# kav-institute/SemanticLiDARUnc

Measured on AMD Instinct MI355X. Metric: range-image scans/sec (64x2048, T=8 MC), higher is better.
Workload: dtype f16 (fp16 activations/weights, fp32 accumulate + epilogue, fp32 logits); 1 GPU; SalsaNext MC-dropout T=8 + entropy/MI map + IoU/ECE accumulation, 8 scans of 64x2048x5 per step per GPU (BASELINE configs[2] shape); T=8, parallelism=scan-sharded x1, mc_schedule=every pass fully recomputed

## Files before the change

semanticlidarunc_amd/csrc/conv2d_h8.hip:

```cpp
#include <stdio.h>
#include "h8_common.h"
#include <cstdlib>

#ifndef H8_M128_OPT_3X3
#define H8_M128_OPT_3X3 15
#endif
#ifndef H8_M128_OPT_2X2
#define H8_M128_OPT_2X2 15
#endif
#ifndef H8_M128_KPC2_DEFAULT
#define H8_M128_KPC2_DEFAULT 0
#endif

namespace {

struct H8Src {
  const uint4* ptr;
  const float* scale;
  int G;
  int gbeg;
  int nb;
  int shuf;
};

struct H8Args {
  H8Src src[SLU_MAX_SRC];
  int nsrc;
  int N, H, W, Gin, Cout, Gout, nmblk, nks;
  const uint4* wpack;
  const float *bias, *bn_a, *bn_b;
  int has_act;
  float slope;
  int out_f32;
  int tiles_x, tiles_y;
  int order;
#ifdef SLU_H8_AB
  int dbg;
#endif
};

struct SrcSel {
  const uint4* ptr;
  const float* scale;
  int G, gl, ns;
};

__device__ __forceinline__ SrcSel select_src(const H8Args& a, const int (&img)[SLU_MAX_SRC], int g) {
  SrcSel p{a.src[0].ptr, a.src[0].scale, a.src[0].G, g, img[0]};
#pragma unroll
  for (int s = 1; s < SLU_MAX_SRC; ++s)
    if (s < a.nsrc && g >= a.src[s].gbeg) p = SrcSel{a.src[s].ptr, a.src[s].scale, a.src[s].G, g - a.src[s].gbeg, img[s]};
  return p;
}

template <int STRIDE>
__device__ __forceinline__ void store_tile(const H8Args& a, const f32x16& acc, const float* se, int cl0, int co0, int hh, bool pix_ok,
                                           size_t n, size_t pix, size_t HW, const void* __restrict__ resid, void* __restrict__ out,
                                           float slope_pre) {
#pragma unroll
  for (int q = 0; q < 4; ++q) {
    float v[4];
#pragma unroll
    for (int k = 0; k < 4; ++k) {
      const int cl = cl0 + 8 * q + 4 * hh + k;
      float t = acc[4 * q + k] + se[cl];
      t = t > 0.0f ? t : t * slope_pre;
      v[k] = t * se[STRIDE + cl] + se[2 * STRIDE + cl];
    }
    const int co = co0 + 8 * q + 4 * hh;
    if (a.out_f32) {
      float* o = reinterpret_cast<float*>(out);
#pragma unroll
      for (int k = 0; k < 4; ++k)
        if (pix_ok && co + k < a.Cout) o[(n * a.Cout + co + k) * HW + pix] = v[k];
    } else {
      const int go = co >> 3;
      const bool ok = pix_ok && go < a.Gout;
      const size_t idx = ok ? ((n * a.Gout + go) * HW + pix) * 2 + hh : 0;
      if (resid) {
        const uint2 rv = reinterpret_cast<const uint2*>(resid)[idx];
        const half2v r0 = __builtin_bit_cast(half2v, rv.x), r1 = __builtin_bit_cast(half2v, rv.y);
        v[0] += (float)r0[0]; v[1] += (float)r0[1]; v[2] += (float)r1[0]; v[3] += (float)r1[1];
      }
      if (ok) reinterpret_cast<uint2*>(out)[idx] = make_uint2(pack2(v[0], v[1]), pack2(v[2], v[3]));
    }
  }
}

template <int STRIDE, bool PRE>
__device__ __forceinline__ void store_tile_full(const H8Args& a, const f32x16& acc, const float* se, int cl0, int go0, int hh, bool pix_ok, size_t n,
                                                size_t pix, size_t HW, const uint2* __restrict__ resid, const uint2 (&rv)[4],
                                                uint2* __restrict__ out, float slope_pre, uintptr_t zero_addr, uintptr_t trash_addr) {
  const float4* se4 = reinterpret_cast<const float4*>(se);
  const float2v sl = {slope_pre, slope_pre};
  const size_t plane2 = HW * 2;
  const size_t idx0 = ((n * a.Gout + go0) * HW + pix) * 2 + hh;
#pragma unroll
  for (int q = 0; q < 4; ++q) {
    const int c4 = (cl0 + 8 * q) / 4 + hh;
    H8Quad t = h8_epilogue(acc, q, se4[c4], se4[STRIDE / 4 + c4], se4[2 * STRIDE / 4 + c4], sl);
    const bool ok = pix_ok && go0 + q < a.Gout;
    const size_t idx = idx0 + q * plane2;
    if (resid) h8_add_resid(t, PRE ? rv[q] : *(ok ? resid + idx : reinterpret_cast<const uint2*>(zero_addr)));
    *(ok ? out + idx : reinterpret_cast<uint2*>(trash_addr)) = pack4(t);
  }
}

template <int STRIDE>
__device__ __forceinline__ void store_tile_swap16(const H8Args& a, const f32x16& acc, const float* se, int cl0, int go0, int hh, bool pix_ok, size_t n,
                                                  size_t pix, size_t HW, const uint2* __restrict__ resid, uint4* __restrict__ out, float slope_pre,
                                                  uintptr_t zero_addr, uintptr_t trash_addr) {
  const float4* se4 = reinterpret_cast<const float4*>(se);
  const float2v sl = {slope_pre, slope_pre};
#pragma unroll
  for (int pr = 0; pr < 2; ++pr) {
    unsigned hw[4];
#pragma unroll
    for (int q2 = 0; q2 < 2; ++q2) {
      const int q = 2 * pr + q2;
      const int c4 = (cl0 + 8 * q) / 4 + hh;
      H8Quad t = h8_epilogue(acc, q, se4[c4], se4[STRIDE / 4 + c4], se4[2 * STRIDE / 4 + c4], sl);
      if (resid) {
        const bool okq = pix_ok && go0 + q < a.Gout;
        h8_add_resid(t, *(okq ? resid + (((n * a.Gout + go0 + q) * HW + pix) * 2 + hh) : reinterpret_cast<const uint2*>(zero_addr)));
      }
      hw[2 * q2] = pack2(t.t0);
      hw[2 * q2 + 1] = pack2(t.t1);
    }
    const uint4 rec = h8_swap16(hw[0], hw[1], hw[2], hw[3]);
    const int go = go0 + 2 * pr + hh;
    *((pix_ok && go < a.Gout) ? out + ((n * a.Gout + go) * HW + pix) : reinterpret_cast<uint4*>(trash_addr)) = rec;
  }
}

#ifdef SLU_H8_PROF
__device__ unsigned long long g_h8_prof[8];
#define H8_PROF_MARK(i)                                         \
  {                                                             \
    const unsigned long long t_now = __builtin_amdgcn_s_memtime(); \
    asm volatile("" ::: "memory");                              \
    prof_acc[i] += t_now - prof_t;                              \
    prof_t = t_now;                                             \
  }
#else
#define H8_PROF_MARK(i)
#endif

constexpr int h8_waves_per_simd(int mb, int nwave, int rpw) { return (mb * rpw >= 8) ? 1 : ((nwave >= 8 || mb >= 2 || rpw >= 2) ? 2 : 3); }

template <int KS, int DIL, int PAD, int MB, int WM, int WN, int RPW, bool SCALED, bool WRES, bool F32OUT, int KPC = 1, int OPT = 0, bool ONE = false>
__global__ __launch_bounds__(64 * WM * WN, h8_waves_per_simd(MB, WM * WN, RPW)) void conv_h8_kernel(const H8Args a, const void* __restrict__ resid,
                                                                                                       void* __restrict__ out) {
  constexpr int NWAVE = WM * WN;
  constexpr int T = KS * KS, TS = KPC * T;
  constexpr int TW = 64, TH = WN * RPW, NB = 2 * RPW;
  constexpr int LW = TW + 2 * PAD, LH = TH + 2 * PAD;
  constexpr int REC = LH * LW;
  constexpr int MBLK = WM * MB;
  constexpr int NREC_B = KPC * 2 * REC, NBLK_B = (NREC_B + 63) / 64;
  constexpr int NB_ALLOC = NBLK_B * 64;
  constexpr int NREC_A = MBLK * TS * 64, NBLK_A = MBLK * TS;
  constexpr int NIB = (NBLK_B + NWAVE - 1) / NWAVE, NIA = (NBLK_A + NWAVE - 1) / NWAVE;
  static_assert(KPC == 1 || (!WRES && !SCALED && MB == 2 && WM == 2 && WN == 4), "multi-K-step chunks: the 8-wave 128-channel configuration only");
  static_assert(OPT == 0 || (MB == 2 && WM == 2 && WN == 4 && !F32OUT), "OPT: the 8-wave 128-channel configuration only");
  static_assert(KPC <= 2, "pc_rc carries 2 bits of channel block");
  static_assert(KPC == 1 || ONE, "multi-K-step chunks: single-source layers only");
  constexpr bool SHUF = SCALED && KS == 3 && DIL == 1 && PAD == 1 && !ONE && KPC == 1;
  static_assert(!SHUF || (WN * RPW) % 2 == 0, "tile rows start on even image rows");

  extern __shared__ __attribute__((aligned(16))) char smem[];
  float* s_epi = reinterpret_cast<float*>(smem);
  uint4* s_scale = reinterpret_cast<uint4*>(s_epi + 3 * MBLK * 32);
  uint4* s_b = s_scale + (SCALED ? 128 : 0);
  uint4* s_a = s_b + 2 * NB_ALLOC;

  const int tid = threadIdx.x, lane = tid & 63, wave = __builtin_amdgcn_readfirstlane(tid >> 6);
  const int wm = wave / WN, wn = wave % WN;
  const bool late_half = wave >= NWAVE / 2;
  const int mblk0 = blockIdx.y * MBLK;
  int t_beg, t_end, t_step = 1;
  {
    const int nwg = gridDim.x, b = blockIdx.x, xcd = b & 7, qq = nwg >> 3, rr = nwg & 7;
    const int w = (xcd < rr ? xcd * (qq + 1) : rr * (qq + 1) + (xcd - rr) * qq) + (b >> 3);
    const long long nt = (long long)a.tiles_x * a.tiles_y * a.N;
    if (a.order) {
      t_step = nwg;
      t_beg = w;
      t_end = w < nt ? w + (int)((nt - w + nwg - 1) / nwg) * nwg : w;
    } else {
      t_beg = (int)(nt * w / nwg);
      t_end = (int)(nt * (w + 1) / nwg);
    }
  }
  t_beg = __builtin_amdgcn_readfirstlane(t_beg);
  t_end = __builtin_amdgcn_readfirstlane(t_end);
  t_step = __builtin_amdgcn_readfirstlane(t_step);
  if (t_beg >= t_end) return;

  if (tid < MBLK * 32) {
    const int co = mblk0 * 32 + tid;
    const bool ok = co < a.Cout;
    H8_FILL_EPI(s_epi, 0, MBLK * 32, tid, ok, co, a.bias, a.bn_a, a.bn_b);
  }

  const int hh = lane >> 5, jj = lane & 31;
  const size_t HW = (size_t)a.H * a.W;
  const float slope_pre = (a.has_act & 3) == 1 ? a.slope : 1.0f;
  const int nks = a.nks;
  const int nchunk = (nks + KPC - 1) / KPC;
  const int a_stride = WRES ? nks * T * 64 : TS * 64;
  const int abase = (wm * MB) * a_stride + lane;
  const int bbase = hh * REC + (wn * RPW) * LW + jj;

  struct TilePos { int tx, ty, x0, y0, n, i0, i1, i2; };
  auto rfl = [](int v) __attribute__((always_inline)) { return __builtin_amdgcn_readfirstlane(v); };
  const int step_tx = rfl(t_step % a.tiles_x), step_ty = rfl((t_step / a.tiles_x) % a.tiles_y), step_n = rfl(t_step / (a.tiles_x * a.tiles_y));
  auto finish = [&](TilePos& p) __attribute__((always_inline)) {
    p.x0 = p.tx * TW;
    p.y0 = p.ty * TH;
    p.i0 = p.i1 = p.i2 = p.n;
    if constexpr (!ONE) {
      if (a.src[0].nb) p.i0 = rfl(p.n % a.src[0].nb);
      if (a.nsrc > 1 && a.src[1].nb) p.i1 = rfl(p.n % a.src[1].nb);
      if (a.nsrc > 2 && a.src[2].nb) p.i2 = rfl(p.n % a.src[2].nb);
    }
  };
  auto decode = [&](int t) __attribute__((always_inline)) {
    TilePos p;
    p.tx = rfl(t % a.tiles_x);
    t /= a.tiles_x;
    p.ty = rfl(t % a.tiles_y);
    p.n = rfl(t / a.tiles_y);
    finish(p);
    return p;
  };
  auto advance = [&](TilePos p) __attribute__((always_inline)) {
    p.tx += step_tx;
    if (p.tx >= a.tiles_x) p.tx -= a.tiles_x, p.ty += 1;
    p.ty += step_ty;
    if (p.ty >= a.tiles_y) p.ty -= a.tiles_y, p.n += 1;
    p.n += step_n;
    finish(p);
    return p;
  };
  static_assert(SLU_MAX_SRC == 3, "TilePos carries one image index per source");
  H8_OPAQUE_ADDR(zero_addr, h8_zero_rec);
  H8_OPAQUE_ADDR(trash_addr, h8_trash_rec);
  int pc_rc[NIB], pc_off[NIB];
#pragma unroll
  for (int i = 0; i < NIB; ++i) {
    const int e = (i * NWAVE + wave) * 64 + lane;
    const int g2 = e / REC;
    const int rem = e - g2 * REC;
    const int r = rem / LW;
    const int c = rem - r * LW;
    pc_rc[i] = r | (c << 8) | ((g2 & (2 * KPC - 1)) << 16) | ((e < NREC_B ? 1 : 0) << 20);
    pc_off[i] = r * a.W + c + (g2 & (2 * KPC - 1)) * (int)HW;
  }
  constexpr int NPIECE = NIB + (WRES ? 0 : NIA);
  constexpr int PPT = (NPIECE + TS - 1) / TS;
  uintptr_t st_b0 = 0, st_b1 = 0;
  bool st_sh = false;
  const int hw4 = (a.H >> 1) * (a.W >> 1), w2 = a.W >> 1;
  int st_g0 = 0;
  bool st_on = false;
  int st_x0 = 0, st_y0 = 0, st_q = 0, st_wave = wave;
  uint4 *st_db = s_b, *st_da = s_a;
  auto stage_begin = [&](const TilePos& tp, int q, int buf) __attribute__((always_inline)) {
    const int img[SLU_MAX_SRC] = {tp.i0, tp.i1, tp.i2};
    long long org = (long long)(tp.y0 - PAD) * a.W + (tp.x0 - PAD);
    st_g0 = 2 * KPC * q;
    if constexpr (SHUF) {
      st_sh = a.src[0].shuf && st_g0 < a.src[0].G;
      if (st_sh) org = 0;
    }
    if constexpr (ONE) {
      st_b0 = reinterpret_cast<uintptr_t>(a.src[0].ptr) + 16 * ((long long)(((size_t)tp.n * a.src[0].G + st_g0) * HW) + org);
      st_b1 = st_b0;
    } else {
      const SrcSel p0 = select_src(a, img, st_g0 < a.Gin ? st_g0 : 0), p1 = select_src(a, img, st_g0 + 1 < a.Gin ? st_g0 + 1 : 0);
      st_b0 = reinterpret_cast<uintptr_t>(p0.ptr) + 16 * ((long long)(((size_t)p0.ns * p0.G + p0.gl) * HW) + org);
      st_b1 = reinterpret_cast<uintptr_t>(p1.ptr) + 16 * ((long long)(((size_t)p1.ns * p1.G + p1.gl) * HW) + org - (long long)HW);
    }
    st_x0 = tp.x0 - PAD;
// ... 332 lines not shown
        x[ks][b] = ok ? v : make_uint4(0u, 0u, 0u, 0u);
      }
    }
    __syncthreads();
    H8_PROF_MARK(0)
    uint4 sw[NW];
#pragma unroll
    for (int i = 0; i < NW; ++i) {
      const int e = tid + i * 256;
      const int m = e / (KSPC * 64);
      const int r = e - m * (KSPC * 64);
      const int ks = r >> 6;
      const bool ok = (NWV % 256 == 0 || e < NWV) && m < a.nmblk && q * KSPC + ks < a.nks;
      const size_t off = ok ? ((size_t)m * a.nks + q * KSPC) * 64 + r : 0;
      sw[i] = a.wpack[off];
      if (!ok) sw[i] = make_uint4(0u, 0u, 0u, 0u);
    }
#pragma unroll
    for (int i = 0; i < NW; ++i) {
      const int e = tid + i * 256;
      if (NWV % 256 == 0 || e < NWV) s_a[e] = sw[i];
    }
#ifdef SLU_H8_PROF
    asm volatile("s_waitcnt lgkmcnt(0)" ::: "memory");
#endif
    H8_PROF_MARK(1)
    __syncthreads();
    H8_PROF_MARK(2)
#pragma unroll
    for (int ks = 0; ks < KSPC; ++ks)
#pragma unroll
      for (int i = 0; i < MB; ++i) {
        const half8 af = __builtin_bit_cast(half8, s_a[(i * KSPC + ks) * 64 + lane]);
#pragma unroll
        for (int b = 0; b < NBW; ++b)
          acc[i][b] = __builtin_amdgcn_mfma_f32_32x32x16_f16(af, __builtin_bit_cast(half8, x[ks][b]), acc[i][b], 0, 0, 0);
      }
#ifdef SLU_H8_PROF
    asm volatile("s_nop 0" ::"v"(acc[MB - 1][NBW - 1][0]));
#endif
    H8_PROF_MARK(3)
  }

  const float slope_pre = (a.has_act & 3) == 1 ? a.slope : 1.0f;
#pragma unroll
  for (int i = 0; i < MB; ++i)
#pragma unroll
    for (int b = 0; b < NBW; ++b)
      store_tile<MB * 32>(a, acc[i][b], s_epi, i * 32, i * 32, hh, live[b], (size_t)nimg[b], (size_t)hw[b], (size_t)HW, resid, out, slope_pre);
#ifdef SLU_H8_PROF
  asm volatile("s_waitcnt vmcnt(0)" ::: "memory");
  H8_PROF_MARK(4)
  if (tid == 0) {
    for (int i = 0; i < 5; ++i) atomicAdd(&g_h8_prof[i], prof_acc[i]);
    atomicAdd(&g_h8_prof[5], 1ull);
  }
#endif
}

constexpr int h8_1x1_res_waves_per_simd(int mb, int nks) { return (mb * nks >= 12) ? 2 : ((mb * nks >= 2) ? 3 : 4); }

template <int MB, int NKS>
__global__ __launch_bounds__(256, h8_1x1_res_waves_per_simd(MB, NKS)) void conv1x1_h8_res_kernel(const H8Args a, const void* __restrict__ resid, void* __restrict__ out) {
  extern __shared__ __attribute__((aligned(16))) char smem[];
  float* s_epi = reinterpret_cast<float*>(smem);
  uint4* s_a = reinterpret_cast<uint4*>(s_epi + 3 * MB * 32);

  const int tid = threadIdx.x, lane = tid & 63, wave = tid >> 6;
  const int hh = lane >> 5, jj = lane & 31;
  const long long HW = (long long)a.H * a.W;
  const long long nblocks = (long long)a.N * HW / 32;

  if (tid < MB * 32) {
    const bool ok = tid < a.Cout;
    H8_FILL_EPI(s_epi, 0, MB * 32, tid, ok, tid, a.bias, a.bn_a, a.bn_b);
  }
  for (int e = tid; e < MB * NKS * 64; e += 256) {
    const int m = e / (NKS * 64);
    const int r = e - m * (NKS * 64);
    const bool ok = m < a.nmblk && (r >> 6) < a.nks;
    s_a[e] = ok ? a.wpack[(size_t)m * a.nks * 64 + r] : make_uint4(0u, 0u, 0u, 0u);
  }
  __syncthreads();

  const float slope_pre = (a.has_act & 3) == 1 ? a.slope : 1.0f;
  const uint2* resid2 = reinterpret_cast<const uint2*>(resid);
  const long long stride = (long long)gridDim.x * 4;
  for (long long pb = (long long)blockIdx.x * 4 + wave; pb < nblocks; pb += stride) {
    const long long pix = pb * 32 + jj;
    const int n = (int)(pix / HW);
    const size_t hw = (size_t)(pix - n * HW);
    int img[SLU_MAX_SRC];
#pragma unroll
    for (int s = 0; s < SLU_MAX_SRC; ++s) img[s] = (s < a.nsrc && a.src[s].nb) ? n % a.src[s].nb : n;
    uint4 x[NKS];
#pragma unroll
    for (int ks = 0; ks < NKS; ++ks) {
      const int g = 2 * ks + hh;
      const bool ok = g < a.Gin;
      const SrcSel p = select_src(a, img, ok ? g : 0);
      const uint4 v = p.ptr[ok ? ((size_t)p.ns * p.G + p.gl) * HW + hw : 0];
      x[ks] = ok ? v : make_uint4(0u, 0u, 0u, 0u);
    }
    uint2 rv[MB][4];
    if (resid) {
#pragma unroll
      for (int i = 0; i < MB; ++i)
#pragma unroll
        for (int q = 0; q < 4; ++q) {
          const int go = i * 4 + q;
          rv[i][q] = go < a.Gout ? resid2[(((size_t)n * a.Gout + go) * HW + hw) * 2 + hh] : make_uint2(0u, 0u);
        }
    }
    f32x16 acc[MB];
#pragma unroll
    for (int i = 0; i < MB; ++i)
#pragma unroll
      for (int r = 0; r < 16; ++r) acc[i][r] = 0.0f;
#pragma unroll
    for (int ks = 0; ks < NKS; ++ks)
#pragma unroll
      for (int i = 0; i < MB; ++i)
        acc[i] = __builtin_amdgcn_mfma_f32_32x32x16_f16(__builtin_bit_cast(half8, s_a[(i * NKS + ks) * 64 + lane]), __builtin_bit_cast(half8, x[ks]),
                                                        acc[i], 0, 0, 0);
#pragma unroll
    for (int i = 0; i < MB; ++i) {
      if (a.out_f32) {
        store_tile<MB * 32>(a, acc[i], s_epi, i * 32, i * 32, hh, true, (size_t)n, hw, (size_t)HW, nullptr, out, slope_pre);
      } else {
#pragma unroll
        for (int q = 0; q < 4; ++q) {
          float v[4];
#pragma unroll
          for (int k = 0; k < 4; ++k) {
            const int cl = i * 32 + 8 * q + 4 * hh + k;
            float t = acc[i][4 * q + k] + s_epi[cl];
            t = t > 0.0f ? t : t * slope_pre;
            v[k] = t * s_epi[MB * 32 + cl] + s_epi[2 * MB * 32 + cl];
          }
          if (resid) {
            const half2v r0 = __builtin_bit_cast(half2v, rv[i][q].x), r1 = __builtin_bit_cast(half2v, rv[i][q].y);
            v[0] += (float)r0[0]; v[1] += (float)r0[1]; v[2] += (float)r1[0]; v[3] += (float)r1[1];
          }
          const int go = i * 4 + q;
          if (go < a.Gout)
            reinterpret_cast<uint2*>(out)[(((size_t)n * a.Gout + go) * HW + hw) * 2 + hh] = make_uint2(pack2(v[0], v[1]), pack2(v[2], v[3]));
          __builtin_amdgcn_sched_barrier(0);
        }
      }
    }
  }
}

template <int MB, int KC, int D>
__global__ __launch_bounds__(512, 2) void gemm1x1_h8_kernel(const H8Args a, const void* __restrict__ resid, void* __restrict__ out) {
  constexpr int NWAVE = 8, MBLK = 2 * MB, TP = 256, NB = 2;
  constexpr int NREC_A = MBLK * KC * 64, NREC_B = 2 * KC * TP;
  constexpr int NPA = MBLK * KC, NPB = 2 * KC * 4;
  constexpr int NIA = (NPA + NWAVE - 1) / NWAVE, NIB = NPB / NWAVE;
  constexpr int NPIECE = NIA + NIB;
  static_assert(NPB % NWAVE == 0 && NPA % NWAVE == 0 && D >= 2 && (D - 2) * NPIECE <= 63, "pieces divide over the waves; vmcnt is 6 bits");

  extern __shared__ __attribute__((aligned(16))) char smem[];
  float* s_epi = reinterpret_cast<float*>(smem);
  uint4* s_b = reinterpret_cast<uint4*>(s_epi + 3 * MBLK * 32);
  uint4* s_a = s_b + D * NREC_B;

  const int tid = threadIdx.x, lane = tid & 63, wave = __builtin_amdgcn_readfirstlane(tid >> 6);
  const int wm = wave >> 2, wn = wave & 3, hh = lane >> 5, jj = lane & 31;
  const size_t HW = (size_t)a.H * a.W;
  const int tiles_per_img = (int)(HW / TP);
  const int ntiles = tiles_per_img * a.N, nch = a.nks / KC;
  const int t_step = gridDim.x, t_beg = (int)blockIdx.x;
  if (t_beg >= ntiles) return;

  if (tid < MBLK * 32) {
    const bool ok = tid < a.Cout;
    H8_FILL_EPI(s_epi, 0, MBLK * 32, tid, ok, tid, a.bias, a.bn_a, a.bn_b);
  }
  H8_OPAQUE_ADDR(zero_addr, h8_zero_rec);
  H8_OPAQUE_ADDR(trash_addr, h8_trash_rec);

  int s_tile = t_beg, s_q = 0, s_slot = 0;
  auto stage_next = [&]() __attribute__((always_inline)) {
    const bool valid = s_tile < ntiles;
    int wv = wave;
    asm volatile("" : "+s"(wv));
    uintptr_t base = zero_addr;
    if (valid) {
      const int n = s_tile / tiles_per_img, p0 = (s_tile - n * tiles_per_img) * TP;
      const int g = 2 * KC * s_q;
      const uint4* ptr = a.src[0].ptr;
      int G = a.src[0].G, gl = g;
#pragma unroll
      for (int s = 1; s < SLU_MAX_SRC; ++s)
        if (s < a.nsrc && g >= a.src[s].gbeg) ptr = a.src[s].ptr, G = a.src[s].G, gl = g - a.src[s].gbeg;
      base = reinterpret_cast<uintptr_t>(ptr) + 16 * (((size_t)n * G + gl) * HW + p0);
    }
    uint4* db = s_b + s_slot * NREC_B;
    uint4* da = s_a + s_slot * NREC_A;
#pragma unroll
    for (int i = 0; i < NIB; ++i) {
      const int p = i * NWAVE + wv;
      const uintptr_t src = (valid && !SLU_ABLATE(a, 1)) ? base + 16 * ((size_t)(p >> 2) * HW + (size_t)((p & 3) * 64 + lane)) : zero_addr;
      SLU_GLDS16(reinterpret_cast<const uint4*>(src), db + p * 64);
    }
#pragma unroll
    for (int i = 0; i < NIA; ++i) {
      const int p = i * NWAVE + wv;
      const int m = p / KC, ks = p - m * KC;
      const uint4* src = (valid && !SLU_ABLATE(a, 2)) ? a.wpack + ((size_t)m * a.nks + KC * s_q + ks) * 64 + lane : reinterpret_cast<const uint4*>(zero_addr);
      SLU_GLDS16(src, da + p * 64);
    }
    asm volatile("" ::: "memory");
    s_slot = s_slot + 1 == D ? 0 : s_slot + 1;
    if (++s_q == nch) s_q = 0, s_tile += t_step;
  };
#pragma unroll
  for (int c = 0; c < D - 1; ++c) stage_next();

  int r_slot = 0;
  const float slope_pre = (a.has_act & 3) == 1 ? a.slope : 1.0f;
  const uint2* resid2 = reinterpret_cast<const uint2*>(resid);
  const int abase = (wm * MB) * KC * 64 + lane;
  const int bbase = hh * TP + wn * 64 + jj;

  for (int tile = t_beg; tile < ntiles; tile += t_step) {
    f32x16 acc[MB][NB];
    h8_zero(acc);
    for (int q = 0; q < nch; ++q) {
      h8_chunk_landed<(D - 2) * NPIECE>();
      stage_next();
      const uint4* sb = s_b + r_slot * NREC_B + bbase;
      const uint4* sa = s_a + r_slot * NREC_A + abase;
      r_slot = r_slot + 1 == D ? 0 : r_slot + 1;
      half8 af[2][MB], bf[2][NB];
      auto read_frags = [&](int set, int ks) __attribute__((always_inline)) {
#pragma unroll
        for (int i = 0; i < MB; ++i) af[set][i] = __builtin_bit_cast(half8, sa[(i * KC + ks) * 64]);
#pragma unroll
        for (int b = 0; b < NB; ++b) bf[set][b] = __builtin_bit_cast(half8, sb[2 * ks * TP + b * 32]);
      };
      read_frags(0, 0);
#pragma unroll
      for (int ks = 0; ks < KC; ++ks) {
        if (ks + 1 < KC) read_frags((ks + 1) & 1, ks + 1);
        __builtin_amdgcn_sched_barrier(0);
        if (!SLU_ABLATE(a, 4)) {
#pragma unroll
          for (int b = 0; b < NB; ++b)
#pragma unroll
            for (int i = 0; i < MB; ++i) acc[i][b] = __builtin_amdgcn_mfma_f32_32x32x16_f16(af[ks & 1][i], bf[ks & 1][b], acc[i][b], 0, 0, 0);
        } else {
#pragma unroll
          for (int i = 0; i < MB; ++i) asm volatile("" ::"v"(af[ks & 1][i]));
#pragma unroll
          for (int b = 0; b < NB; ++b) asm volatile("" ::"v"(bf[ks & 1][b]));
        }
        __builtin_amdgcn_sched_barrier(0);
      }
    }
    {
      const int n = tile / tiles_per_img, p0 = (tile - n * tiles_per_img) * TP;
#pragma unroll
      for (int i = 0; i < MB; ++i) {
        const int ml = wm * MB + i;
#pragma unroll
        for (int b = 0; b < NB; ++b) {
          const size_t pix = (size_t)p0 + wn * 64 + b * 32 + jj;
          store_tile_swap16<MBLK * 32>(a, acc[i][b], s_epi, ml * 32, ml * 4, hh, true, (size_t)n, pix, HW, resid2, reinterpret_cast<uint4*>(out), slope_pre,
                                       zero_addr, trash_addr);
          __builtin_amdgcn_sched_barrier(0);
        }
      }
    }
  }
  asm volatile("s_waitcnt vmcnt(0)" ::: "memory");
}

__global__ void pack_h8_kernel(const float* __restrict__ w, int cout, int cin, int ks, int nks, size_t total, uint4* __restrict__ out) {
  const int T = ks * ks;
  for (size_t e = (size_t)blockIdx.x * blockDim.x + threadIdx.x; e < total; e += (size_t)gridDim.x * blockDim.x) {
    const int lane = (int)(e & 63);
    size_t r = e >> 6;
    const int tap = (int)(r % T);
    r /= T;
    const int k = (int)(r % nks);
    const int m = (int)(r / nks);
    const int co = m * 32 + (lane & 31);
    float x[8];
#pragma unroll
    for (int j = 0; j < 8; ++j) {
      const int ci = k * 16 + 8 * (lane >> 5) + j;
      x[j] = (co < cout && ci < cin) ? w[((size_t)co * cin + ci) * T + tap] : 0.0f;
    }
    out[e] = make_uint4(pack2(x[0], x[1]), pack2(x[2], x[3]), pack2(x[4], x[5]), pack2(x[6], x[7]));
  }
}

__global__ __launch_bounds__(256) void nchw_to_h8_kernel(const float* __restrict__ x, const float* __restrict__ scale, uint4* __restrict__ y, int N,
                                                         int C, int G, size_t HW) {
  const size_t total = (size_t)N * G * HW;
  for (size_t e = (size_t)blockIdx.x * blockDim.x + threadIdx.x; e < total; e += (size_t)gridDim.x * blockDim.x) {
    const size_t pix = e % HW;
    const size_t ng = e / HW;
    const int g = (int)(ng % G);
    const size_t n = ng / G;
    float v[8];
#pragma unroll
    for (int k = 0; k < 8; ++k) {
      const int c = g * 8 + k;
      v[k] = c < C ? x[(n * C + c) * HW + pix] * (scale ? scale[n * C + c] : 1.0f) : 0.0f;
    }
    y[e] = make_uint4(pack2(v[0], v[1]), pack2(v[2], v[3]), pack2(v[4], v[5]), pack2(v[6], v[7]));
  }
}

__global__ __launch_bounds__(256) void h8_to_nchw_kernel(const uint4* __restrict__ x, float* __restrict__ y, int N, int C, int G, size_t HW) {
  const size_t total = (size_t)N * G * HW;
  for (size_t e = (size_t)blockIdx.x * blockDim.x + threadIdx.x; e < total; e += (size_t)gridDim.x * blockDim.x) {
    const size_t pix = e % HW;
    const size_t ng = e / HW;
    const int g = (int)(ng % G);
    const size_t n = ng / G;
    const half8 h = __builtin_bit_cast(half8, x[e]);
#pragma unroll
    for (int k = 0; k < 8; ++k) {
      const int c = g * 8 + k;
      if (c < C) y[(n * C + c) * HW + pix] = (float)h[k];
    }
  }
}

__global__ __launch_bounds__(256) void avgpool3s2_h8_kernel(const uint4* __restrict__ x, const float* __restrict__ scale, uint4* __restrict__ y,
                                                            int N, int G, int H, int W, int OH, int OW, int in_batch, int tiles) {
  const int g = (int)(blockIdx.x / (unsigned)tiles);
  const int ox = (int)(blockIdx.x - (unsigned)g * (unsigned)tiles) * 256 + (int)threadIdx.x;
  if (ox >= OW) return;
  const int ix = 2 * ox - 1;
  const bool xin = ox >= 1 && ix + 2 < W;
  for (int n = (int)blockIdx.z; n < N; n += (int)gridDim.z) {
    const size_t ni = in_batch ? (size_t)(n % in_batch) : (size_t)n;
    const uint4* img = x + (ni * G + g) * (size_t)H * W;
    float s[8];
    if (scale) {
      const float4 s0 = *reinterpret_cast<const float4*>(scale + ((size_t)n * G + g) * 8);
      const float4 s1 = *reinterpret_cast<const float4*>(scale + ((size_t)n * G + g) * 8 + 4);
      s[0] = s0.x; s[1] = s0.y; s[2] = s0.z; s[3] = s0.w;
      s[4] = s1.x; s[5] = s1.y; s[6] = s1.z; s[7] = s1.w;
    } else {
#pragma unroll
      for (int k = 0; k < 8; ++k) s[k] = 1.0f;
    }
    for (int oy = (int)blockIdx.y; oy < OH; oy += (int)gridDim.y) {
      const int iy = 2 * oy - 1;
      float acc[8];
#pragma unroll
      for (int k = 0; k < 8; ++k) acc[k] = 0.0f;
      if (xin && oy >= 1 && iy + 2 < H) {
        const uint4* p = img + (size_t)iy * W + ix;
#pragma unroll
        for (int i = 0; i < 3; ++i)
#pragma unroll
          for (int j = 0; j < 3; ++j) {
            const half8 h = __builtin_bit_cast(half8, p[(size_t)i * W + j]);
#pragma unroll
            for (int k = 0; k < 8; ++k) acc[k] += (float)h[k];
          }
      } else {
#pragma unroll
        for (int i = 0; i < 3; ++i)
#pragma unroll
          for (int j = 0; j < 3; ++j) {
            const bool ok = iy + i >= 0 && iy + i < H && ix + j >= 0 && ix + j < W;
            const half8 h = __builtin_bit_cast(half8, img[ok ? (size_t)(iy + i) * W + (ix + j) : 0]);
#pragma unroll
            for (int k = 0; k < 8; ++k) acc[k] += ok ? (float)h[k] : 0.0f;
          }
      }
#pragma unroll
      for (int k = 0; k < 8; ++k) acc[k] = acc[k] * s[k] / 9.0f;
      y[(((size_t)n * G + g) * OH + oy) * OW + ox] =
          make_uint4(pack2(acc[0], acc[1]), pack2(acc[2], acc[3]), pack2(acc[4], acc[5]), pack2(acc[6], acc[7]));
    }
  }
}

__global__ __launch_bounds__(256) void pixel_shuffle_h8_kernel(const uint4* __restrict__ x, const float* __restrict__ s_in,
                                                               const float* __restrict__ s_out, uint4* __restrict__ y, int N, int Gi, int Go, int H,
                                                               int W) {
  const size_t total = (size_t)N * Go * H * W;
  const size_t HWi = (size_t)H * W;
  const int OW = 2 * W;
  for (size_t e = (size_t)blockIdx.x * blockDim.x + threadIdx.x; e < total; e += (size_t)gridDim.x * blockDim.x) {
    const int w = (int)(e % W);
    size_t r = e / W;
    const int h = (int)(r % H);
    r /= H;
    const int go = (int)(r % Go);
    const size_t n = r / Go;
    float v[4][8];
#pragma unroll
    for (int q = 0; q < 4; ++q) {
      const int gi = 4 * go + q;
      const bool ok = gi < Gi;
      const half8 rec = __builtin_bit_cast(half8, ok ? x[(n * Gi + gi) * HWi + (size_t)h * W + w] : make_uint4(0u, 0u, 0u, 0u));
#pragma unroll
      for (int slot = 0; slot < 8; ++slot) {
        float t = (float)rec[slot];
        if (ok && s_in) t *= s_in[n * Gi * 8 + gi * 8 + slot];
        v[slot & 3][2 * q + (slot >> 2)] = t;
      }
    }
    if (s_out) {
#pragma unroll
      for (int k = 0; k < 8; ++k) {
        const int co = 8 * go + k;
        const float so = co < 2 * Gi ? s_out[n * (Gi * 2) + co] : 0.0f;
#pragma unroll
        for (int sub = 0; sub < 4; ++sub) v[sub][k] *= so;
      }
    }
#pragma unroll
    for (int sub = 0; sub < 4; ++sub) {
      const size_t o = ((n * Go + go) * (size_t)(2 * H) + (2 * h + (sub >> 1))) * OW + 2 * w + (sub & 1);
      y[o] = make_uint4(pack2(v[sub][0], v[sub][1]), pack2(v[sub][2], v[sub][3]), pack2(v[sub][4], v[sub][5]), pack2(v[sub][6], v[sub][7]));
    }
  }
}

// ... 304 lines not shown
}

bool ring3_ok(const slu_conv_h8_desc* d, const H8Args& a) {
  static const bool off = [] { const char* e = getenv("SLU_H8_RING3"); return e && e[0] == '0'; }();
  if (off || d->ksize != 3 || d->pad != d->dil || (d->dil != 1 && d->dil != 2) || a.nsrc < 1 || a.nsrc > 2) return false;
  int gsum = 0;
  for (int s = 0; s < a.nsrc; ++s) {
    if ((a.src[s].scale && !a.src[s].shuf) || a.src[s].nb) return false;
    gsum += a.src[s].G;
  }
  if (a.src[0].shuf && !(a.nsrc == 2 && a.Gin == 10 && a.src[0].G == 2)) return false;
  if (gsum != a.Gin || (a.nsrc == 2 && (a.src[0].G & 1)) || a.out_f32 || d->resid || (a.has_act & ~1)) return false;
  if ((a.has_act & 1) && !(a.slope >= 0.0f && a.slope <= 1.0f)) return false;
  return (a.Cout == 32 || a.Cout == 64) && ((a.Gin == 4 || a.Gin == 8) || (a.Gin == 10 && a.Cout == 32 && d->dil == 1));
}

int launch_ring3_any(const H8Args& a, const slu_conv_h8_desc* d, const SluEmit& e) {
  const int mb = a.Cout / 32, nks = a.Gin / 2;
  if (nks == 5) return launch_ring3<1, 1, 5, 1, 4>(a, d, e);
  if (mb == 2 && nks == 4) return d->dil == 1 ? launch_ring3<1, 2, 4, 1, 3>(a, d, e) : launch_ring3<2, 2, 4, 1, 3>(a, d, e);
  if (mb == 2 && nks == 2) return d->dil == 1 ? launch_ring3<1, 2, 2, 2, 3>(a, d, e) : launch_ring3<2, 2, 2, 1, 3>(a, d, e);
  if (mb == 1 && nks == 4) return d->dil == 1 ? launch_ring3<1, 1, 4, 2, 3>(a, d, e) : launch_ring3<2, 1, 4, 1, 3>(a, d, e);
  return d->dil == 1 ? launch_ring3<1, 1, 2, 2, 3>(a, d, e) : launch_ring3<2, 1, 2, 2, 3>(a, d, e);
}

constexpr size_t WRES_MAX_BYTES = 24 * 1024;

template <int KS, int DIL, int PAD, int MB, int WM, int WN, int RPW, bool SCALED>
int launch_h8(H8Args& a, const slu_conv_h8_desc* d, const SluEmit& e) {
  const size_t wbytes = (size_t)WM * MB * a.nks * KS * KS * 64 * 16;
  if (wbytes <= WRES_MAX_BYTES) return launch_h8_k<KS, DIL, PAD, MB, WM, WN, RPW, SCALED, true>(a, d, e);
  return launch_h8_k<KS, DIL, PAD, MB, WM, WN, RPW, SCALED, false>(a, d, e);
}

inline long long wg_count(const H8Args& a, int th, int mblk) {
  return (long long)a.N * ((a.H + th - 1) / th) * ((a.W + 63) / 64) * ((a.nmblk + mblk - 1) / mblk);
}

enum { CFG_M32_TH16 = 0, CFG_M64_TH16, CFG_M128_TH8, CFG_M32_TH8, CFG_M64_TH8, CFG_M128_TH4, CFG_M32_TH4, CFG_M64_TH4, CFG_COUNT };

int choose_h8(const H8Args& a) {
  const long long want = 256;
  static const int forced = [] { const char* e = getenv("SLU_H8_CFG"); return e ? atoi(e) : -1; }();
  if (forced >= 0 && forced < CFG_COUNT) return forced;
  if (a.nmblk >= 4) {
    if (a.H >= 8 && wg_count(a, 8, 4) >= want) return CFG_M128_TH8;
    if (wg_count(a, 4, 4) >= want) return CFG_M128_TH4;
    if (wg_count(a, 4, 2) >= want) return CFG_M64_TH4;
    return CFG_M32_TH4;
  }
  if (a.nmblk >= 2) {
    if (a.H >= 16 && wg_count(a, 16, 2) >= want) return CFG_M64_TH16;
    if (a.H >= 8 && wg_count(a, 8, 2) >= want) return CFG_M64_TH8;
    if (wg_count(a, 4, 2) >= want) return CFG_M64_TH4;
    return CFG_M32_TH4;
  }
  if (a.H >= 16 && wg_count(a, 16, 1) >= want) return CFG_M32_TH16;
  if (a.H >= 8 && wg_count(a, 8, 1) >= want) return CFG_M32_TH8;
  return CFG_M32_TH4;
}

int g_h8_opt = [] { const char* e = getenv("SLU_H8_OPT"); return e ? atoi(e) : -1; }();
int g_h8_kpc2 = [] { const char* e = getenv("SLU_H8_KPC2"); return e ? atoi(e) : H8_M128_KPC2_DEFAULT; }();

constexpr size_t h8_m128_weight_bytes(int nks, int T) { return (size_t)4 * nks * T * 64 * 16; }

inline bool h8_one_plain_source(const H8Args& a) { return a.nsrc == 1 && a.src[0].nb == 0 && !a.src[0].scale; }

template <int KS, int DIL, int PAD, bool SCALED>
int launch_h8_m128(H8Args& a, const slu_conv_h8_desc* d, const SluEmit& e) {
  if (h8_m128_weight_bytes(a.nks, KS * KS) <= WRES_MAX_BYTES) return launch_h8_k<KS, DIL, PAD, 2, 2, 4, 2, SCALED, true>(a, d, e);
  if constexpr (!SCALED) {
    if (h8_one_plain_source(a)) {
      if constexpr (KS == 2) {
        if (g_h8_kpc2 && a.nks >= 2) {
#ifdef SLU_H8_AB
          if (g_h8_opt == 0) return launch_h8_k<KS, DIL, PAD, 2, 2, 4, 2, false, false, false, 2, 0, true>(a, d, e);
#endif
          return launch_h8_k<KS, DIL, PAD, 2, 2, 4, 2, false, false, false, 2, H8_M128_OPT_2X2, true>(a, d, e);
        }
      }
#ifdef SLU_H8_AB
      switch (g_h8_opt) {
        case 0: return launch_h8_k<KS, DIL, PAD, 2, 2, 4, 2, false, false, false, 1, 0, true>(a, d, e);
        case 8: return launch_h8_k<KS, DIL, PAD, 2, 2, 4, 2, false, false, false, 1, 8, true>(a, d, e);
        case 15: return launch_h8_k<KS, DIL, PAD, 2, 2, 4, 2, false, false, false, 1, 15, true>(a, d, e);
        case 100: return launch_h8_k<KS, DIL, PAD, 2, 2, 4, 2, false, false, false, 1, 0, false>(a, d, e);
      }
#endif
      return launch_h8_k<KS, DIL, PAD, 2, 2, 4, 2, false, false, false, 1, KS == 2 ? H8_M128_OPT_2X2 : H8_M128_OPT_3X3, true>(a, d, e);
    }
  }
  return launch_h8_k<KS, DIL, PAD, 2, 2, 4, 2, SCALED, false>(a, d, e);
}

template <int KS, int DIL, int PAD, bool SCALED>
int launch_h8_tiles(H8Args& a, const slu_conv_h8_desc* d, int cfg, const SluEmit& e) {
  switch (cfg) {
    case CFG_M32_TH16: return launch_h8<KS, DIL, PAD, 1, 1, 8, 2, SCALED>(a, d, e);
    case CFG_M64_TH16: return launch_h8<KS, DIL, PAD, 2, 1, 8, 2, SCALED>(a, d, e);
    case CFG_M128_TH8: return launch_h8_m128<KS, DIL, PAD, SCALED>(a, d, e);
    case CFG_M32_TH8:  return launch_h8<KS, DIL, PAD, 1, 1, 4, 2, SCALED>(a, d, e);
    case CFG_M64_TH8:  return launch_h8<KS, DIL, PAD, 2, 1, 4, 2, SCALED>(a, d, e);
    case CFG_M128_TH4: return launch_h8<KS, DIL, PAD, 2, 2, 2, 2, SCALED>(a, d, e);
    case CFG_M32_TH4:  return launch_h8<KS, DIL, PAD, 1, 1, 4, 1, SCALED>(a, d, e);
    case CFG_M64_TH4:  return launch_h8<KS, DIL, PAD, 2, 1, 4, 1, SCALED>(a, d, e);
  }
  return SLU_EUNSUPPORTED;
}

template <int KS, int DIL, int PAD>
int launch_h8_family(H8Args& a, const slu_conv_h8_desc* d, int cfg, bool scaled, const SluEmit& e) {
  return scaled ? launch_h8_tiles<KS, DIL, PAD, true>(a, d, cfg, e) : launch_h8_tiles<KS, DIL, PAD, false>(a, d, cfg, e);
}

template <int MB, int NBW>
int launch_h8_1x1(H8Args& a, const slu_conv_h8_desc* d, const SluEmit& e) {
  constexpr size_t lds = (size_t)MB * 4 * 64 * 16 + (size_t)3 * MB * 32 * 4;
  const long long nblocks = (long long)a.N * a.H * a.W / 32;
  const long long gx = (nblocks + 4 * NBW - 1) / (4 * NBW);
  if (gx <= 0 || gx > 0x7fffffffLL) return SLU_EUNSUPPORTED;
  if (e.name) return slu_emit_name(e, "conv1x1_h8_kernel<%d, %d>", MB, NBW);
  hipLaunchKernelGGL((conv1x1_h8_kernel<MB, NBW>), dim3((unsigned)gx), dim3(256), lds, e.st, a, d->resid, d->out);
  SLU_CHECK_LAUNCH();
}

template <int MB, int NKS>
int launch_h8_1x1_res(H8Args& a, const slu_conv_h8_desc* d, const SluEmit& e) {
  constexpr size_t lds = (size_t)MB * NKS * 64 * 16 + (size_t)3 * MB * 32 * 4;
  const long long nblocks = (long long)a.N * a.H * a.W / 32;
  long long gx = 256 * h8_1x1_res_waves_per_simd(MB, NKS);
  if (gx * 4 > nblocks) gx = (nblocks + 3) / 4;
  if (gx <= 0) return SLU_EUNSUPPORTED;
  if (e.name) return slu_emit_name(e, "conv1x1_h8_res_kernel<%d, %d>", MB, NKS);
  hipLaunchKernelGGL((conv1x1_h8_res_kernel<MB, NKS>), dim3((unsigned)gx), dim3(256), lds, e.st, a, d->resid, d->out);
  SLU_CHECK_LAUNCH();
}

template <int MB>
int launch_h8_1x1_res_nks(H8Args& a, const slu_conv_h8_desc* d, const SluEmit& e) {
  switch (a.nks) {
    case 1:  return launch_h8_1x1_res<MB, 1>(a, d, e);
    case 2:  return launch_h8_1x1_res<MB, 2>(a, d, e);
    case 5: case 6:   return launch_h8_1x1_res<MB, 6>(a, d, e);
    case 10: case 12: return launch_h8_1x1_res<MB, 12>(a, d, e);
  }
  return -1;
}

constexpr int GEMM1X1_KC = 4, GEMM1X1_D256 = 2, GEMM1X1_D128 = 3;
bool gemm1x1_ok(const slu_conv_h8_desc* d, const H8Args& a) {
  static const bool off = [] { const char* e = getenv("SLU_H8_GEMM1X1"); return e && e[0] == '0'; }();
  static const bool all = [] { const char* e = getenv("SLU_H8_GEMM1X1"); return e && e[0] == '2'; }();
  if (off || d->ksize != 1 || d->pad != 0 || a.out_f32 || (a.Cout != 256 && !(all && a.Cout == 128))) return false;
  if (((long long)a.H * a.W) % 256 || a.nks % GEMM1X1_KC || a.Gin != 2 * a.nks) return false;
  if ((a.has_act & ~1) || ((a.has_act & 1) && !(a.slope >= 0.0f && a.slope <= 1.0f))) return false;
  for (int s = 0; s < a.nsrc; ++s)
    if (a.src[s].scale || a.src[s].nb || a.src[s].G % (2 * GEMM1X1_KC)) return false;
  return (long long)a.N * a.H * a.W / 256 <= 0x7fffffffLL;
}

template <int MB, int D>
int launch_gemm1x1(H8Args& a, const slu_conv_h8_desc* d, const SluEmit& e) {
  constexpr int KC = GEMM1X1_KC, MBLK = 2 * MB;
  constexpr size_t lds = (size_t)3 * MBLK * 32 * 4 + (size_t)D * (2 * KC * 256) * 16 + (size_t)D * (MBLK * KC * 64) * 16;
  static_assert(lds <= 160 * 1024, "gemm1x1 LDS");
  const long long nt = (long long)a.N * a.H * a.W / 256;
  const long long gx = nt < 256 ? nt : 256;
  if (e.name) return slu_emit_name(e, "gemm1x1_h8_kernel<%d, %d, %d>", MB, KC, D);
  static SluLdsGrant grant;
  return slu_launch_lds(gemm1x1_h8_kernel<MB, KC, D>, dim3((unsigned)gx), dim3(512), lds, e.st, grant, a, d->resid, d->out);
}

bool any_scale(const slu_conv_h8_desc* d) {
  for (int s = 0; s < d->nsrc; ++s)
    if (d->src[s].scale) return true;
  return false;
}

bool stream_ok(const slu_conv_h8_desc* d, const H8Args& a) {
  return d->ksize == 1 && d->pad == 0 && a.nmblk <= 8 && ((long long)a.H * a.W) % 32 == 0 && !any_scale(d);
}

int conv_h8_dispatch(const slu_conv_h8_desc* d, const SluEmit& e) {
  H8Args a{};
  const int rc = fill_h8(d, a);
  if (rc != SLU_OK) return rc;
  if (a.src[0].shuf) {
    if (ring3_ok(d, a)) {
      const int rc2 = launch_ring3_any(a, d, e);
      if (rc2 != -1) return rc2;
    }
    if (!any_scale(d) || d->ksize != 3 || d->dil != 1 || d->pad != 1 || a.out_f32) return SLU_EUNSUPPORTED;
    return launch_h8_family<3, 1, 1>(a, d, choose_h8(a), true, e);
  }
  if (gemm1x1_ok(d, a)) return a.Cout == 128 ? launch_gemm1x1<2, GEMM1X1_D128>(a, d, e) : launch_gemm1x1<4, GEMM1X1_D256>(a, d, e);
  if (stream_ok(d, a)) {
    if (a.nmblk <= 2) {
      const int rc2 = a.nmblk == 1 ? launch_h8_1x1_res_nks<1>(a, d, e) : launch_h8_1x1_res_nks<2>(a, d, e);
      if (rc2 != -1) return rc2;
    }
    if (a.nmblk == 1) return launch_h8_1x1<1, 2>(a, d, e);
    if (a.nmblk == 2) return launch_h8_1x1<2, 2>(a, d, e);
    if (a.nmblk <= 4) return launch_h8_1x1<4, 1>(a, d, e);
    return launch_h8_1x1<8, 1>(a, d, e);
  }
  if (ring3_ok(d, a)) {
    const int rc2 = launch_ring3_any(a, d, e);
    if (rc2 != -1) return rc2;
  }
  const bool sc = any_scale(d);
  if (a.out_f32) {
    if (d->ksize != 1 || d->dil != 1 || d->pad != 0 || sc) return SLU_EUNSUPPORTED;
    return launch_h8_k<1, 1, 0, 1, 1, 4, 1, false, false, true>(a, d, e);
  }
  const int cfg = choose_h8(a);
  if (d->ksize == 1 && d->dil == 1 && d->pad == 0) return launch_h8_family<1, 1, 0>(a, d, cfg, sc, e);
  if (d->ksize == 3 && d->dil == 1 && d->pad == 1) return launch_h8_family<3, 1, 1>(a, d, cfg, sc, e);
  if (d->ksize == 3 && d->dil == 2 && d->pad == 2) return launch_h8_family<3, 2, 2>(a, d, cfg, sc, e);
  if (d->ksize == 2 && d->dil == 2 && d->pad == 1) return launch_h8_family<2, 2, 1>(a, d, cfg, sc, e);
  return SLU_EUNSUPPORTED;
}

}

extern "C" size_t slu_packed_weight_bytes_h8(int cout, int cin, int ksize) {
  if (cout <= 0 || cin <= 0 || ksize <= 0) return 0;
  const size_t nmblk = (cout + 31) / 32, nks = (cin + 15) / 16;
  return nmblk * nks * (size_t)(ksize * ksize) * 64 * 16;
}

extern "C" int slu_pack_conv_weight_h8(const float* w, int cout, int cin, int ksize, void* out, slu_stream_t stream) {
  if (!w || !out) return SLU_EINVAL;
  const size_t bytes = slu_packed_weight_bytes_h8(cout, cin, ksize);
  if (bytes == 0) return SLU_EINVAL;
  const size_t total = bytes / 16;
  hipLaunchKernelGGL(pack_h8_kernel, dim3(grid_for(total)), dim3(256), 0, slu_stream(stream), w, cout, cin, ksize, (cin + 15) / 16, total,
                     reinterpret_cast<uint4*>(out));
  SLU_CHECK_LAUNCH();
}

extern "C" int slu_conv2d_h8_fwd(const slu_conv_h8_desc* d, slu_stream_t stream) { return conv_h8_dispatch(d, SluEmit{slu_stream(stream), nullptr, 0}); }

extern "C" int slu_conv2d_h8_kernel_name(const slu_conv_h8_desc* d, char* buf, size_t n) {
  return buf ? conv_h8_dispatch(d, SluEmit{nullptr, buf, n}) : SLU_EINVAL;
}

#ifdef SLU_H8_AB
extern "C" void slu_h8_dev_set_opt(int opt, int kpc2) { g_h8_opt = opt; g_h8_kpc2 = kpc2; }
#endif

#ifdef SLU_H8_PROF
extern "C" int slu_h8_prof_read(unsigned long long* out8) {
  if (hipMemcpyFromSymbol(out8, HIP_SYMBOL(g_h8_prof), sizeof(unsigned long long) * 8) != hipSuccess) return SLU_ELAUNCH;
  unsigned long long z[8] = {};
  return hipMemcpyToSymbol(HIP_SYMBOL(g_h8_prof), z, sizeof(z)) == hipSuccess ? SLU_OK : SLU_ELAUNCH;
}
#endif

extern "C" int slu_nchw_to_h8(const float* x, const float* scale, void* y, int N, int C, int H, int W, slu_stream_t stream) {
  if (!x || !y || N <= 0 || C <= 0 || H <= 0 || W <= 0 || ((uintptr_t)y & 15)) return SLU_EINVAL;
  const int G = (C + 7) / 8;
  const size_t total = (size_t)N * G * H * W;
  hipLaunchKernelGGL(nchw_to_h8_kernel, dim3(grid_for(total)), dim3(256), 0, slu_stream(stream), x, scale, reinterpret_cast<uint4*>(y), N, C, G,
                     (size_t)H * W);
  SLU_CHECK_LAUNCH();
}

extern "C" int slu_h8_to_nchw(const void* x, float* y, int N, int C, int H, int W, slu_stream_t stream) {
  if (!x || !y || N <= 0 || C <= 0 || H <= 0 || W <= 0 || ((uintptr_t)x & 15)) return SLU_EINVAL;
  const int G = (C + 7) / 8;
  const size_t total = (size_t)N * G * H * W;
  hipLaunchKernelGGL(h8_to_nchw_kernel, dim3(grid_for(total)), dim3(256), 0, slu_stream(stream), reinterpret_cast<const uint4*>(x), y, N, C, G,
                     (size_t)H * W);
  SLU_CHECK_LAUNCH();
}

extern "C" int slu_avgpool3s2_h8(const void* x, const float* scale, void* y, int N, int in_batch, int G, int H, int W, slu_stream_t stream) {
  if (!x || !y || N <= 0 || in_batch < 0 || G <= 0 || H <= 0 || W <= 0 || (((uintptr_t)x | (uintptr_t)y | (uintptr_t)scale) & 15)) return SLU_EINVAL;
  const int OH = (H + 1) / 2, OW = (W + 1) / 2;
  const int tiles = (OW + 255) / 256;
  if ((long long)tiles * G > 0x7fffffffLL) return SLU_EUNSUPPORTED;
  const dim3 grid((unsigned)(tiles * G), (unsigned)(OH < 65535 ? OH : 65535), (unsigned)(N < 65535 ? N : 65535));
  hipLaunchKernelGGL(avgpool3s2_h8_kernel, grid, dim3(256), 0, slu_stream(stream), reinterpret_cast<const uint4*>(x), scale,
                     reinterpret_cast<uint4*>(y), N, G, H, W, OH, OW, in_batch, tiles);
  SLU_CHECK_LAUNCH();
}

extern "C" int slu_pixel_shuffle_h8(const void* x, const float* scale_in, const float* scale_out, void* y, int N, int Gin, int H, int W,
                                    slu_stream_t stream) {
  if (!x || !y || N <= 0 || Gin <= 0 || H <= 0 || W <= 0 || (((uintptr_t)x | (uintptr_t)y) & 15)) return SLU_EINVAL;
  const int Go = (Gin * 2 + 7) / 8;
  const size_t total = (size_t)N * Go * H * W;
  hipLaunchKernelGGL(pixel_shuffle_h8_kernel, dim3(grid_for(total)), dim3(256), 0, slu_stream(stream), reinterpret_cast<const uint4*>(x), scale_in,
                     scale_out, reinterpret_cast<uint4*>(y), N, Gin, Go, H, W);
  SLU_CHECK_LAUNCH();
}
```

Measured before the change: 714.7 scans/s.

## Prefetch residual ahead of epilogue in 1x1 GEMM and route concat128 convs to it

The 1x1 GEMM kernel now issues residual-tensor loads with inline asm during the last K chunk and waits on them only before the epilogue. This overlaps residual fetch latency with the final MFMA work. Stores use precomputed 32-bit offsets from a scalar base, and a new size guard keeps those offsets within range. The GEMM path is also widened to cover 128-channel three-source concat convs with a residual. The change adds hand-managed vmcnt waits that depend on exact load counts, plus extra register pressure from holding residuals. An env var keeps the old kernel available.

Measured after the change: 730.7 scans/s, median of 6. 2.2% higher.

```diff
diff --git a/semanticlidarunc_amd/csrc/conv2d_h8.hip b/semanticlidarunc_amd/csrc/conv2d_h8.hip
--- a/semanticlidarunc_amd/csrc/conv2d_h8.hip
+++ b/semanticlidarunc_amd/csrc/conv2d_h8.hip
@@ -130,6 +130,29 @@
     const uint4 rec = h8_swap16(hw[0], hw[1], hw[2], hw[3]);
     const int go = go0 + 2 * pr + hh;
     *((pix_ok && go < a.Gout) ? out + ((n * a.Gout + go) * HW + pix) : reinterpret_cast<uint4*>(trash_addr)) = rec;
+  }
+}
+
+template <int STRIDE, bool RES>
+__device__ __forceinline__ void gemm_store_tile(const f32x16& acc, const float* se, int cl0, int hh, const u32x4v (&res)[2], char* obase, unsigned vo,
+                                                unsigned plane2, float slope_pre) {
+  const float4* se4 = reinterpret_cast<const float4*>(se);
+  const float2v sl = {slope_pre, slope_pre};
+#pragma unroll
+  for (int pr = 0; pr < 2; ++pr) {
+    uint4 rw = make_uint4(0u, 0u, 0u, 0u);
+    if constexpr (RES) rw = h8_swap16(res[pr].x, res[pr].y, res[pr].z, res[pr].w);
+    unsigned hw[4];
+#pragma unroll
+    for (int q2 = 0; q2 < 2; ++q2) {
+      const int q = 2 * pr + q2;
+      const int c4 = (cl0 + 8 * q) / 4 + hh;
+      H8Quad t = h8_epilogue(acc, q, se4[c4], se4[STRIDE / 4 + c4], se4[2 * STRIDE / 4 + c4], sl);
+      if constexpr (RES) h8_add_resid(t, q2 ? make_uint2(rw.z, rw.w) : make_uint2(rw.x, rw.y));
+      hw[2 * q2] = pack2(t.t0);
+      hw[2 * q2 + 1] = pack2(t.t1);
+    }
+    *reinterpret_cast<uint4*>(obase + (size_t)pr * plane2 + vo) = h8_swap16(hw[0], hw[1], hw[2], hw[3]);
   }
 }
 
@@ -768,8 +791,8 @@
   }
 }
 
-template <int MB, int KC, int D>
-__global__ __launch_bounds__(512, 2) void gemm1x1_h8_kernel(const H8Args a, const void* __restrict__ resid, void* __restrict__ out) {
+template <int MB, int KC, int D, bool AHEAD, bool RES>
+__device__ __forceinline__ void gemm1x1_h8_body(const H8Args& a, const void* __restrict__ resid, void* __restrict__ out) {
   constexpr int NWAVE = 8, MBLK = 2 * MB, TP = 256, NB = 2;
   constexpr int NREC_A = MBLK * KC * 64, NREC_B = 2 * KC * TP;
   constexpr int NPA = MBLK * KC, NPB = 2 * KC * 4;
@@ -837,15 +860,39 @@
 
   int r_slot = 0;
   const float slope_pre = (a.has_act & 3) == 1 ? a.slope : 1.0f;
-  const uint2* resid2 = reinterpret_cast<const uint2*>(resid);
+  [[maybe_unused]] const uint2* resid2 = reinterpret_cast<const uint2*>(resid);
   const int abase = (wm * MB) * KC * 64 + lane;
   const int bbase = hh * TP + wn * 64 + jj;
+
+  static_assert(!AHEAD || MB == 2 || MB == 4, "the residual waits name 8 registers per set");
+  const unsigned plane = (unsigned)(HW * 16);
+  unsigned voff[NB];
+#pragma unroll
+  for (int b = 0; b < NB; ++b) voff[b] = (unsigned)(hh * HW * 16) + (unsigned)((wn * 64 + b * 32 + jj) * 16);
+  unsigned long long rbase = 0;
+  auto load_resid = [&](u32x4v (&r)[2][NB][2], int i0) __attribute__((always_inline)) {
+#pragma unroll
+    for (int i = 0; i < 2; ++i)
+#pragma unroll
+      for (int b = 0; b < NB; ++b)
+#pragma unroll
+        for (int pr = 0; pr < 2; ++pr) {
+          const unsigned long long base = rbase + (unsigned long long)((wm * MB + i0 + i) * 4 + 2 * pr) * plane;
+          asm volatile("global_load_dwordx4 %0, %1, %2" : "=&v"(r[i][b][pr]) : "v"(voff[b]), "s"(base) : "memory");
+        }
+  };
 
   for (int tile = t_beg; tile < ntiles; tile += t_step) {
     f32x16 acc[MB][NB];
     h8_zero(acc);
+    u32x4v ra[2][NB][2], rb[2][NB][2];
+    const int n = tile / tiles_per_img, p0 = (tile - n * tiles_per_img) * TP;
+    const size_t tile16 = 16 * ((size_t)n * a.Gout * HW + p0);
+    if constexpr (AHEAD) rbase = reinterpret_cast<unsigned long long>(resid) + tile16;
     for (int q = 0; q < nch; ++q) {
       h8_chunk_landed<(D - 2) * NPIECE>();
+      if constexpr (AHEAD && RES)
+        if (q == nch - 1) load_resid(ra, 0);
       stage_next();
       const uint4* sb = s_b + r_slot * NREC_B + bbase;
       const uint4* sa = s_a + r_slot * NREC_A + abase;
@@ -876,8 +923,36 @@
         __builtin_amdgcn_sched_barrier(0);
       }
     }
-    {
-      const int n = tile / tiles_per_img, p0 = (tile - n * tiles_per_img) * TP;
+    if constexpr (AHEAD) {
+      char* obase = reinterpret_cast<char*>(out) + tile16;
+      {
+        auto blocks = [&](const u32x4v (&r)[2][NB][2], int i0) __attribute__((always_inline)) {
+#pragma unroll
+          for (int i = 0; i < 2; ++i)
+#pragma unroll
+            for (int b = 0; b < NB; ++b) {
+              gemm_store_tile<MBLK * 32, RES>(acc[i0 + i][b], s_epi, (wm * MB + i0 + i) * 32, hh, r[i][b], obase + (size_t)((wm * MB + i0 + i) * 4) * plane,
+                                              voff[b], 2 * plane, slope_pre);
+              __builtin_amdgcn_sched_barrier(0);
+            }
+        };
+        if constexpr (RES)
+          asm volatile("s_waitcnt vmcnt(%8)"
+                       : "+v"(ra[0][0][0]), "+v"(ra[0][0][1]), "+v"(ra[0][1][0]), "+v"(ra[0][1][1]), "+v"(ra[1][0][0]), "+v"(ra[1][0][1]),
+                         "+v"(ra[1][1][0]), "+v"(ra[1][1][1])
+                       : "n"(NPIECE));
+        if constexpr (RES && MB == 4) load_resid(rb, 2);
+        blocks(ra, 0);
+        if constexpr (MB == 4) {
+          if constexpr (RES)
+            asm volatile("s_waitcnt vmcnt(%8)"
+                         : "+v"(rb[0][0][0]), "+v"(rb[0][0][1]), "+v"(rb[0][1][0]), "+v"(rb[0][1][1]), "+v"(rb[1][0][0]), "+v"(rb[1][0][1]),
+                           "+v"(rb[1][1][0]), "+v"(rb[1][1][1])
+                         : "n"(2 * NB * 2));
+          blocks(rb, 2);
+        }
+      }
+    } else {
 #pragma unroll
       for (int i = 0; i < MB; ++i) {
         const int ml = wm * MB + i;
@@ -892,6 +967,16 @@
     }
   }
   asm volatile("s_waitcnt vmcnt(0)" ::: "memory");
+}
+
+template <int MB, int KC, int D>
+__global__ __launch_bounds__(512, 2) void gemm1x1_h8_kernel(const H8Args a, const void* __restrict__ resid, void* __restrict__ out) {
+  if (resid) gemm1x1_h8_body<MB, KC, D, true, true>(a, resid, out);
+  else gemm1x1_h8_body<MB, KC, D, true, false>(a, resid, out);
+}
+template <int MB, int KC, int D>
+__global__ __launch_bounds__(512, 2) void gemm1x1_h8_kernel_v1(const H8Args a, const void* __restrict__ resid, void* __restrict__ out) {
+  gemm1x1_h8_body<MB, KC, D, false, false>(a, resid, out);
 }
 
 __global__ void pack_h8_kernel(const float* __restrict__ w, int cout, int cin, int ks, int nks, size_t total, uint4* __restrict__ out) {
@@ -1502,11 +1587,13 @@
 bool gemm1x1_ok(const slu_conv_h8_desc* d, const H8Args& a) {
   static const bool off = [] { const char* e = getenv("SLU_H8_GEMM1X1"); return e && e[0] == '0'; }();
   static const bool all = [] { const char* e = getenv("SLU_H8_GEMM1X1"); return e && e[0] == '2'; }();
-  if (off || d->ksize != 1 || d->pad != 0 || a.out_f32 || (a.Cout != 256 && !(all && a.Cout == 128))) return false;
+  const bool concat128 = a.Cout == 128 && d->resid && a.nsrc == 3 && a.nks == 24;
+  if (off || d->ksize != 1 || d->pad != 0 || a.out_f32 || (a.Cout != 256 && !(a.Cout == 128 && (all || concat128)))) return false;
   if (((long long)a.H * a.W) % 256 || a.nks % GEMM1X1_KC || a.Gin != 2 * a.nks) return false;
   if ((a.has_act & ~1) || ((a.has_act & 1) && !(a.slope >= 0.0f && a.slope <= 1.0f))) return false;
   for (int s = 0; s < a.nsrc; ++s)
     if (a.src[s].scale || a.src[s].nb || a.src[s].G % (2 * GEMM1X1_KC)) return false;
+  if (16LL * a.Gout * a.H * a.W > 0xffffffffLL) return false;
   return (long long)a.N * a.H * a.W / 256 <= 0x7fffffffLL;
 }
 
@@ -1517,8 +1604,10 @@
   static_assert(lds <= 160 * 1024, "gemm1x1 LDS");
   const long long nt = (long long)a.N * a.H * a.W / 256;
   const long long gx = nt < 256 ? nt : 256;
-  if (e.name) return slu_emit_name(e, "gemm1x1_h8_kernel<%d, %d, %d>", MB, KC, D);
-  static SluLdsGrant grant;
+  static const bool v1 = [] { const char* v = getenv("SLU_GEMM1X1_RES_AHEAD"); return v && v[0] == '0'; }();
+  if (e.name) return slu_emit_name(e, v1 ? "gemm1x1_h8_kernel_v1<%d, %d, %d>" : "gemm1x1_h8_kernel<%d, %d, %d>", MB, KC, D);
+  static SluLdsGrant grant, grant_v1;
+  if (v1) return slu_launch_lds(gemm1x1_h8_kernel_v1<MB, KC, D>, dim3((unsigned)gx), dim3(512), lds, e.st, grant_v1, a, d->resid, d->out);
   return slu_launch_lds(gemm1x1_h8_kernel<MB, KC, D>, dim3((unsigned)gx), dim3(512), lds, e.st, grant, a, d->resid, d->out);
 }
 
```
